# jermp/sshash

Hardware: AMD Instinct MI355X
Metric: k-mer Lookups/sec (batched random queries, bit-exact ids) (higher is better)
Workload: dtype u64

## Files before the change

### sshash_amd/csrc/streaming.hip

```cpp
#include <hip/hip_runtime.h>
#include <sys/stat.h>

#include <algorithm>
#include <atomic>
#include <cstring>
#include <exception>
#include <stdexcept>
#include <thread>

#include "engine.hpp"
#include "hooks.hpp"
#include "reads.hpp"
#include "replica.hpp"
#include "segments.hpp"

namespace sshash_amd {

namespace {

template <int W, bool CANON>
__device__ __forceinline__ hit_t seed_lookup(dict_view const& d, skew_part_dev const* __restrict__ skew,
                                             kmer_w<W> const& x, kmer_w<W> const& x_rc, minimizer_t mf, minimizer_t mr) {
    if constexpr (CANON) {
        if (mf.value < mr.value) return probe_canonical<W, true>(d, skew, x, x_rc, mf);
        if (mr.value < mf.value) return probe_canonical<W, true>(d, skew, x, x_rc, mr);
        hit_t h = probe_canonical<W, true>(d, skew, x, x_rc, mf);
        if (!h.found) h = probe_canonical<W, true>(d, skew, x, x_rc, mr);
        return h;
    } else {
        hit_t h = probe_regular<W, true>(d, skew, x, mf);
        if (!h.found) {
            const bool mf_found = h.minimizer_found;
            h = probe_regular<W, true>(d, skew, x_rc, mr);
            h.orientation = -1;
            h.minimizer_found = h.minimizer_found || mf_found;
        }
        return h;
    }
}

__device__ __forceinline__ uint64_t wave_sum(uint64_t v) {
    for (int o = 32; o > 0; o >>= 1) v += __shfl_down(v, o, 64);
    return v;
}

__device__ __forceinline__ bool continues_run(uint64_t id_before, uint64_t sid_before, int ori_before, uint64_t id, uint64_t sid) {
    return id_before != INVALID_U64 && sid_before == sid && id == id_before + uint64_t(int64_t(ori_before));
}

__device__ __forceinline__ void block_report(uint64_t c_kmers, uint64_t c_invalid, uint64_t c_negative, uint64_t c_searches,
                                             uint64_t c_extensions, uint64_t* __restrict__ report) {
    __shared__ uint64_t partial[4][5];
    c_kmers = wave_sum(c_kmers);
    c_invalid = wave_sum(c_invalid);
    c_negative = wave_sum(c_negative);
    c_searches = wave_sum(c_searches);
    c_extensions = wave_sum(c_extensions);
    if ((threadIdx.x & 63) == 0) {
        uint64_t* mine = partial[threadIdx.x >> 6];
        mine[0] = c_kmers;
        mine[1] = c_invalid;
        mine[2] = c_negative;
        mine[3] = c_searches;
        mine[4] = c_extensions;
    }
    __syncthreads();
    if (threadIdx.x != 0) return;
    uint64_t t[5];
    for (int j = 0; j < 5; ++j) t[j] = partial[0][j] + partial[1][j] + partial[2][j] + partial[3][j];
    if (t[0] == 0) return;
    atomicAdd(reinterpret_cast<unsigned long long*>(report + 0), (unsigned long long)t[0]);
    atomicAdd(reinterpret_cast<unsigned long long*>(report + 1), (unsigned long long)(t[3] + t[4]));
    atomicAdd(reinterpret_cast<unsigned long long*>(report + 2), (unsigned long long)t[2]);
    atomicAdd(reinterpret_cast<unsigned long long*>(report + 3), (unsigned long long)t[1]);
    atomicAdd(reinterpret_cast<unsigned long long*>(report + 4), (unsigned long long)t[3]);
    atomicAdd(reinterpret_cast<unsigned long long*>(report + 5), (unsigned long long)t[4]);
}


__global__ void __launch_bounds__(256)
stream_pack_kernel(const char* __restrict__ bases, const uint64_t total_bases, uint16_t* __restrict__ packed, uint8_t* __restrict__ okay) {
    const uint64_t t = uint64_t(blockIdx.x) * blockDim.x + threadIdx.x;
    const uint64_t at = 8 * t;
    if (at >= total_bases) return;
    uint64_t v = 0;
    if (at + 8 <= total_bases && ((reinterpret_cast<uintptr_t>(bases) + at) & 7) == 0) {
        v = *reinterpret_cast<const uint64_t*>(bases + at);
    } else {
        for (uint32_t b = 0; b < 8 && at + b < total_bases; ++b) v |= uint64_t(uint8_t(bases[at + b])) << (8 * b);
    }
    uint64_t two = (v >> 1) & 0x0303030303030303ULL;
    two = (two | (two >> 6)) & 0x000F000F000F000FULL;
    two = (two | (two >> 12)) & 0x000000FF000000FFULL;
    two = two | (two >> 24);
    const uint64_t u = v & 0xDFDFDFDFDFDFDFDFULL;
    auto nonzero = [](uint64_t z) { return ((z & 0x7F7F7F7F7F7F7F7FULL) + 0x7F7F7F7F7F7F7F7FULL) | z; };
    uint64_t ok = ~(nonzero(u ^ 0x4141414141414141ULL) & nonzero(u ^ 0x4343434343434343ULL) & nonzero(u ^ 0x4747474747474747ULL) &
                    nonzero(u ^ 0x5454545454545454ULL)) & 0x8080808080808080ULL;
    ok >>= 7;
    ok |= ok >> 7;
    ok |= ok >> 14;
    ok |= ok >> 28;
    packed[t] = uint16_t(two);
    okay[t] = uint8_t(ok);
}

__device__ __forceinline__ uint64_t first_invalid_base(const uint64_t* __restrict__ okay, uint64_t from, uint64_t end) {
    uint64_t p = from;
    while (p < end) {
        const uint64_t bad = ~okay[p >> 6] >> (p & 63u);
        if (bad) {
            p += uint64_t(__builtin_ctzll(bad));
            break;
        }
        p = (p | 63u) + 1;
    }
    return p < end ? p : end;
}

__device__ __forceinline__ uint64_t first_valid_base(const uint64_t* __restrict__ okay, uint64_t from, uint64_t end) {
    uint64_t p = from;
    while (p < end) {
        const uint64_t good = okay[p >> 6] >> (p & 63u);
        if (good) {
            p += uint64_t(__builtin_ctzll(good));
            break;
        }
        p = (p | 63u) + 1;
    }
    return p < end ? p : end;
}

__device__ __forceinline__ uint64_t read_bases32(const uint64_t* __restrict__ packed, uint64_t p) {
    const uint64_t i = p >> 5;
    return funnel_shr(packed[i], packed[i + 1], 2 * (uint32_t(p) & 31u));
}

template <int W>
__device__ __forceinline__ void string_bases32(dict_view const& d, uint64_t p, uint64_t& bases, uint64_t& marks) {
    const uint32_t rel = uint32_t(p) & 31u;
    if constexpr (W == 1) {
        const uint4* A = reinterpret_cast<const uint4*>(d.granules) + 2 * (p >> 5);
        const uint4 q0 = A[0], q1 = A[1];
        bases = funnel_shr(uint64_t(q0.x) | (uint64_t(q0.y) << 32), uint64_t(q0.z) | (uint64_t(q0.w) << 32), 2 * rel);
        marks = (uint64_t(q1.x) | (uint64_t(q1.y) << 32)) >> rel;
    } else {
        const uint4* G = reinterpret_cast<const uint4*>(d.granules) + (p >> 5);
        const uint4 g0 = G[0], g1 = G[1];
        bases = funnel_shr(uint64_t(g0.z) | (uint64_t(g0.w) << 32), uint64_t(g1.z) | (uint64_t(g1.w) << 32), 2 * rel);
        marks = (uint64_t(g0.y) | (uint64_t(g1.y) << 32)) >> rel;
    }
}

struct run_step_t {
    uint64_t s, marks, read;
    uint32_t have;
};

template <int W>
__device__ __forceinline__ run_step_t run_step_load(dict_view const& d, const uint64_t* __restrict__ packed, uint64_t off, bool forward,
                                                    uint64_t b, uint64_t run) {
    run_step_t t;
    const uint64_t top = off - run;
    t.have = forward || top >= 32 ? 32u : uint32_t(top);
    string_bases32<W>(d, forward ? off + d.k + run : top - t.have, t.s, t.marks);
    t.read = read_bases32(packed, b + run);
    return t;
}

__device__ __forceinline__ uint32_t run_step_length(run_step_t const& t, bool forward) {
    const uint64_t along = forward ? t.s : revcomp_word(t.s << ((2 * (32 - t.have)) & 63u));
    const uint64_t diff = along ^ t.read;
    const uint32_t same = diff ? uint32_t(__builtin_ctzll(diff)) >> 1 : 32u;
    const uint32_t gate = forward ? uint32_t(__brev(uint32_t(t.marks))) : uint32_t((t.marks >> 1) << (32 - t.have));
    const uint32_t inside = gate ? uint32_t(__builtin_clz(gate)) : 32u;
    const uint32_t step = same < inside ? same : inside;
    return step < t.have ? step : t.have;
}

template <int W>
__device__ __forceinline__ uint64_t extend_run(dict_view const& d, const uint64_t* __restrict__ packed, uint64_t off, int ori, uint64_t b,
                                               uint64_t room, run_step_t t) {
    const bool forward = ori > 0;
    uint64_t run = 0;
    for (;;) {
        uint64_t step = run_step_length(t, forward);
        if (step > room - run) step = room - run;
        run += step;
        if (step < 32 || run >= room) break;
        t = run_step_load<W>(d, packed, off, forward, b, run);
    }
    return run;
}

__device__ __forceinline__ void row_flush(uint64_t* __restrict__ row, bool partial, uint32_t& c_invalid, uint32_t& c_negative, uint32_t& c_searches,
                                          uint32_t& c_extensions) {
    const uint64_t s = c_searches, e = c_extensions;
    if (partial) {
        row[1] += s + e;
        row[2] += c_negative;
        row[3] += c_invalid;
        row[4] += s;
        row[5] += e;
    } else {
        row[1] = s + e;
        row[2] = c_negative;
        row[3] = c_invalid;
        row[4] = s;
        row[5] = e;
    }
    c_invalid = c_negative = c_searches = c_extensions = 0;
}

#ifndef SSHASH_STREAM_WAVES
#define SSHASH_STREAM_WAVES 5
#endif
enum : int { STREAM_TOTALS = 0, STREAM_ROWS = 1, STREAM_RUN_COUNTS = 2, STREAM_RUN_RECORDS = 3, STREAM_COVER = 4, STREAM_DEPTH = 5 };

__device__ __forceinline__ void run_record_store(dict_view const& d, run_sink const& sink, const uint64_t* __restrict__ begins, uint64_t r,
                                                 uint64_t cursor, uint64_t at, uint64_t off, uint32_t sid, int ori, uint64_t n) {
    if (cursor >= sink.capacity || cursor >= sink.run_offsets[r + 1]) return;
    const uint64_t kmer_id = off - uint64_t(sid) * (d.k - 1), in_string = off - d.endpoints[sid];
    const uint32_t read_pos = uint32_t(at - begins[r]), length = uint32_t(n) | (ori > 0 ? 0u : 0x80000000u);
    uint4* const rec = static_cast<uint4*>(sink.records) + 2 * cursor;
    rec[0] = make_uint4(uint32_t(kmer_id), uint32_t(kmer_id >> 32), sid, 0u);
    rec[1] = make_uint4(uint32_t(in_string), uint32_t(in_string >> 32), read_pos, length);
}

__device__ __forceinline__ void cover_mark(uint64_t* __restrict__ cover, uint64_t lo, uint64_t hi) {
    const uint64_t w0 = lo >> 6, w1 = (hi - 1) >> 6;
    const unsigned long long first = ~0ULL << (lo & 63u), last = ~0ULL >> (63u - (uint32_t(hi - 1) & 63u));
    unsigned long long* const words = reinterpret_cast<unsigned long long*>(cover);
    if (w0 == w1) {
        (void)__hip_atomic_fetch_or(words + w0, first & last, __ATOMIC_RELAXED, __HIP_MEMORY_SCOPE_AGENT);
        return;
    }
    (void)__hip_atomic_fetch_or(words + w0, first, __ATOMIC_RELAXED, __HIP_MEMORY_SCOPE_AGENT);
    for (uint64_t w = w0 + 1; w < w1; ++w) words[w] = ~0ULL;
    (void)__hip_atomic_fetch_or(words + w1, last, __ATOMIC_RELAXED, __HIP_MEMORY_SCOPE_AGENT);
}

__device__ __forceinline__ void cover_mark_run(dict_view const& d, run_sink const& sink, uint64_t off, uint32_t sid, int ori, uint64_t n) {
    const uint64_t kmer_id = off - uint64_t(sid) * (d.k - 1);
    const uint64_t lo = ori > 0 ? kmer_id : kmer_id + 1 - n;
    cover_mark(static_cast<uint64_t*>(sink.records), lo, lo + n);
}

__device__ __forceinline__ void depth_mark_run(dict_view const& d, run_sink const& sink, uint64_t off, uint32_t sid, int ori, uint64_t n) {
    const uint64_t kmer_id = off - uint64_t(sid) * (d.k - 1);
    const uint64_t lo = ori > 0 ? kmer_id : kmer_id + 1 - n, hi = lo + n;
    uint32_t* const deltas = static_cast<uint32_t*>(sink.records);
    (void)__hip_atomic_fetch_add(deltas + lo, 1u, __ATOMIC_RELAXED, __HIP_MEMORY_SCOPE_AGENT);
    if (hi < d.num_kmers) (void)__hip_atomic_fetch_add(deltas + hi, ~0u, __ATOMIC_RELAXED, __HIP_MEMORY_SCOPE_AGENT);
}

template <int W, bool CANON, bool SK, int MODE>
__global__ void __launch_bounds__(256, SSHASH_STREAM_WAVES)
streaming_run_kernel(const dict_view d, const skew_part_dev* __restrict__ skew, const uint64_t* __restrict__ packed,
                     const uint64_t* __restrict__ okay, const uint64_t* __restrict__ begins, const uint64_t* __restrict__ ends, const uint64_t n_reads,
                     const uint64_t reads_per_wave, const uint32_t move_out_every, uint64_t* __restrict__ report, const run_sink sink) {
    constexpr bool PER_READ = MODE == STREAM_ROWS, COUNT_RUNS = MODE == STREAM_RUN_COUNTS, RECORDS = MODE == STREAM_RUN_RECORDS, COVER = MODE == STREAM_COVER,
                   DEPTH = MODE == STREAM_DEPTH;
    __shared__ uint4 stage[SK ? 4 * 256 : 1];
    uint4* const wave_stage = stage + (SK ? (threadIdx.x >> 6) * 256 : 0);
    __shared__ unsigned long long moved_out[4][5];
    uint32_t c_invalid = 0, c_negative = 0, c_searches = 0, c_extensions = 0;
    const uint32_t k = d.k;
    const uint32_t lane = threadIdx.x & 63u;
    unsigned long long* const wave_moved_out = moved_out[threadIdx.x >> 6];
    if constexpr (!PER_READ && !RECORDS) {
        if (lane < 5) wave_moved_out[lane] = 0;
    }
    const uint64_t wave = uint64_t(blockIdx.x) * (blockDim.x >> 6) + (threadIdx.x >> 6);
    uint64_t next = wave * reads_per_wave, last = next + reads_per_wave;
    if (next > n_reads) next = n_reads;
    if (last > n_reads) last = n_reads;
    uint64_t cur = 0, rd_end = 0, inv = 0;
    bool pending = false;
    uint64_t off = 0;
    int ori = 1;
    bool neg_unknown_mini = false;
    uint64_t prev_f = 0, prev_r = 0;
    constexpr uint32_t WALK_CHOICE = 7u, WALK_COMPACT = 8u, WALK_VISITED = 16u, WALK_BACK_SHIFT = 8u, WALK_NO_RETURN = 7u;
    constexpr uint32_t WALK_LASTS_SHIFT = 16u, WALK_LASTS = 63u;
    constexpr uint32_t WALK_INLINE = 32u, WALK_HEAVY_BACK_SHIFT = 11u, WALK_HEAVY_SHIFT = 24u, WALK_HEAVY = 63u, WALK_HEAVY_PENDING = 1u << 30;
    constexpr uint32_t WALK_HEAVY_FIELDS = (7u << WALK_HEAVY_BACK_SHIFT) | (WALK_HEAVY << WALK_HEAVY_SHIFT) | WALK_HEAVY_PENDING;
    bool walking = false;
    kmer_w<W> x = kmer_zero<W>(), x_rc = kmer_zero<W>();
    sk_key_t kk{};
    uint64_t on = 0, on_a = 0;
    uint32_t where = 0;
    uint32_t turns = 0;
    constexpr uint32_t ROW_NONE = ~0u, ROW_PARTIAL = 1u << 31;
    uint32_t my_row = ROW_NONE;
    uint32_t n_runs = 0, hit_sid = 0;
    uint64_t cursor = 0;
    const uint64_t wave_first = wave * reads_per_wave;
    uint64_t* const wave_rows = report + wave * reads_per_wave * 6;
#ifdef SSHASH_STREAM_STATS
    unsigned long long st_turns = 0, st_fresh = 0, st_walk = 0, st_ext = 0, st_slot1 = 0, st_inv = 0, st_idle = 0, st_full = 0, st_short = 0;
    uint64_t st_kept_lane = 0;
#define STAT(var, pred) var += (unsigned long long)__popcll(__ballot(pred))
#else
#define STAT(var, pred) (void)0
#endif
    for (;;) {
#ifdef SSHASH_STREAM_STATS
        ++st_turns;
#endif
        if (++turns >= move_out_every) {
            turns = 0;
            if constexpr (PER_READ) {
                if (my_row != ROW_NONE) {
                    row_flush(wave_rows + uint64_t(my_row & ~ROW_PARTIAL) * 6, (my_row & ROW_PARTIAL) != 0, c_invalid, c_negative, c_searches, c_extensions);
                    my_row |= ROW_PARTIAL;
                }
            } else if constexpr (!RECORDS) {
                const uint64_t i = wave_sum(c_invalid), n = wave_sum(c_negative), f = wave_sum(c_searches), e = wave_sum(c_extensions);
                if (lane == 0) {
                    wave_moved_out[0] += i;
                    wave_moved_out[1] += n;
                    wave_moved_out[2] += f;
                    wave_moved_out[3] += e;
                }
                c_invalid = c_negative = c_searches = c_extensions = 0;
            }
        }
        STAT(st_ext, pending);
        if (pending) {
            const uint64_t b = cur + k - 1, valid_end = inv < rd_end ? inv : rd_end;
            const uint64_t run = extend_run<W>(d, packed, off, ori, b, valid_end - b, run_step_load<W>(d, packed, off, ori > 0, b, 0));
            if constexpr (COVER) cover_mark_run(d, sink, off, hit_sid, ori, run + 1);
            if constexpr (DEPTH) depth_mark_run(d, sink, off, hit_sid, ori, run + 1);
            if constexpr (RECORDS) {
                run_record_store(d, sink, begins, wave_first + my_row, cursor, cur - 1, off, hit_sid, ori, run + 1);
                ++cursor;
            } else if (run >> 15) {
                if constexpr (PER_READ) {
                    uint64_t* const row = wave_rows + uint64_t(my_row & ~ROW_PARTIAL) * 6;
                    row_flush(row, (my_row & ROW_PARTIAL) != 0, c_invalid, c_negative, c_searches, c_extensions);
                    my_row |= ROW_PARTIAL;
                    row[1] += run;
                    row[5] += run;
                } else {
                    atomicAdd(wave_moved_out + 3, (unsigned long long)run);
                }
            } else {
                c_extensions += uint32_t(run);
            }
            cur += run;
            if (run) where &= ~WALK_HEAVY_FIELDS;
        }
        pending = false;
        const bool want = !walking && cur + k > rd_end;
        const uint64_t wants = __ballot(want);
        if constexpr (PER_READ) {
            if (want && my_row != ROW_NONE) {
                row_flush(wave_rows + uint64_t(my_row & ~ROW_PARTIAL) * 6, (my_row & ROW_PARTIAL) != 0, c_invalid, c_negative, c_searches, c_extensions);
                my_row = ROW_NONE;
            }
        }
        if constexpr (COUNT_RUNS) {
            if (want && my_row != ROW_NONE) {
                sink.run_offsets[wave_first + my_row] = n_runs;
                n_runs = 0;
                my_row = ROW_NONE;
            }
        }
        if (wants != 0 && next < last) {
            const uint64_t rank = uint64_t(__popcll(wants & ((uint64_t(1) << lane) - 1)));
            if (want && rank < last - next) {
                const uint64_t r = next + rank;
                cur = begins[r];
                rd_end = ends[r];
                if constexpr (PER_READ) {
                    uint64_t* const row = report + r * 6;
                    const uint64_t kmers = rd_end - cur >= k ? rd_end - cur - k + 1 : 0;
                    row[0] = kmers;
                    if (kmers) {
                        my_row = uint32_t(r - wave * reads_per_wave);
                    } else {
                        row[1] = row[2] = row[3] = row[4] = row[5] = 0;
                    }
                } else if constexpr (COUNT_RUNS) {
                    if (rd_end - cur >= k) {
                        atomicAdd(wave_moved_out + 4, (unsigned long long)(rd_end - cur - k + 1));
                        my_row = uint32_t(r - wave_first);
                    } else {
                        sink.run_offsets[r] = 0;
                    }
                } else if constexpr (RECORDS) {
                    my_row = uint32_t(r - wave_first);
                    cursor = sink.run_offsets[r];
                } else {
                    if (rd_end - cur >= k) atomicAdd(wave_moved_out + 4, (unsigned long long)(rd_end - cur - k + 1));
                }
                inv = first_invalid_base(okay, cur, rd_end);
                neg_unknown_mini = false;
                where = 0;
            }
            const uint64_t taken = uint64_t(__popcll(wants));
            next = taken < last - next ? next + taken : last;
        }
        bool live = cur + k <= rd_end;
        if (next >= last && __ballot(live) == 0) break;
        uint32_t c_invalid_turn = 0;
        STAT(st_inv, live && cur + k > inv);
        while (live && cur + k > inv) {
            const uint64_t nv = first_valid_base(okay, inv + 1, rd_end);
            const uint64_t last_over_it = nv - 1 < rd_end - k ? nv - 1 : rd_end - k;
            const uint64_t over = last_over_it - cur + 1;
            if ((over + c_invalid_turn) >> 15) {
                if constexpr (PER_READ) {
                    uint64_t* const row = wave_rows + uint64_t(my_row & ~ROW_PARTIAL) * 6;
                    row_flush(row, (my_row & ROW_PARTIAL) != 0, c_invalid, c_negative, c_searches, c_extensions);
                    my_row |= ROW_PARTIAL;
                    row[3] += over;
                } else if constexpr (!RECORDS) {
                    atomicAdd(wave_moved_out + 0, (unsigned long long)over);
                }
            } else {
                c_invalid_turn += uint32_t(over);
            }
            cur = nv;
            inv = first_invalid_base(okay, nv, rd_end);
            neg_unknown_mini = false;
            where = 0;
            live = cur + k <= rd_end;
        }
        c_invalid += c_invalid_turn;
        const uint64_t valid_end = inv < rd_end ? inv : rd_end;
        uint64_t ahead_f = 0, ahead_r = 0;
        bool table = false;
        STAT(st_fresh, live && !walking);
        STAT(st_walk, live && walking);
        STAT(st_idle, !live);
        if (live && !walking) {
            const uint64_t i = cur >> 5;
            const uint32_t sh = 2 * (uint32_t(cur) & 31u);
            const uint64_t w0 = packed[i], w1 = packed[i + 1];
            x.w[0] = funnel_shr(w0, w1, sh);
            if constexpr (W == 2) x.w[1] = funnel_shr(w1, packed[i + 2], sh);
            x = kmer_take_chars<W>(x, k);
            x_rc = kmer_revcomp<W>(x, k);
            if constexpr (SK) {
                const uint32_t sm = d.sk.m, hashed = sm < 12 ? sm : 12;
                ahead_f = read_bases32(packed, cur + k - sm + 1);
                ahead_r = read_bases32(packed, cur + k + 1 - hashed);
                const uint32_t heavy_left = (where >> WALK_HEAVY_SHIFT) & WALK_HEAVY;
                STAT(st_short, heavy_left != 0);
                if (heavy_left) {
                    kk.pos = kk.rc ? kk.pos + 1 : kk.pos - 1;
                    table = true;
                    on = sk_kmer_key<W>(x, x_rc);
                    const uint32_t back = (where >> WALK_HEAVY_BACK_SHIFT) & 7u;
                    where = WALK_VISITED | WALK_COMPACT | (back << WALK_BACK_SHIFT) | (back << WALK_HEAVY_BACK_SHIFT) | ((heavy_left - 1) << WALK_HEAVY_SHIFT);
                } else {
                    kk = sk_key<W>(x, x_rc, k, sm);
                    table = sk_usable(d, kk);
                    on = kk.key;
                    where = (WALK_NO_RETURN << WALK_BACK_SHIFT) | (WALK_LASTS << WALK_LASTS_SHIFT);
                }
                on_a = sk_hash_a(on);
            }
        }
        if constexpr (SK) {
            if (live && walking && (!(where & WALK_VISITED) || (where & WALK_HEAVY_PENDING))) {
                const uint32_t sm = d.sk.m, hashed = sm < 12 ? sm : 12;
                ahead_f = read_bases32(packed, cur + k - sm + 1);
                ahead_r = read_bases32(packed, cur + k + 1 - hashed);
            }
        }
        bool settled = false, found = false;
        if constexpr (SK) {
            const bool need = table || walking;
            const uint32_t c = where & WALK_CHOICE;
            const bool compact = (where & WALK_COMPACT) != 0;
            uint32_t bucket = 0;
            if (need) bucket = compact ? d.sk.num_buckets + sk_choice_of(on, on_a, c, d.sk.kmer_buckets) : sk_choice_of(on, on_a, c, d.sk.num_buckets);
            sk_stage_lines<W, true>(d, bucket, 0u, need, wave_stage, compact);
            if (need) {
                const uint4* mine = wave_stage + (lane & 3u) * 64 + (lane >> 2) * 4;
                sk_query_t<W> Q = sk_make_query<W>(x, x_rc, kk, uint32_t(on_a) & 0xFFFFFFu);
                fast_t r = fast_unsettled(false);
                sk_bucket_flags flags;
                flags.go_on = 0;
                flags.second_used = false;
                bool marker = false, seen = false, inline_seen = false;
                uint32_t lasts = 0xFFFFu;
                if (!compact) {
                    sk_examine_slot_tracking<W, true, true>(d, Q, c, [mine](uint32_t i) { return mine[i]; }, r, seen, marker, flags, lasts, inline_seen);
                    STAT(st_slot1, r.outcome == FAST_MISS && flags.second_used);
                    if (r.outcome == FAST_MISS && flags.second_used) {
                        if constexpr (W == 1) {
                            sk_examine_slot_tracking<W, false, true>(d, Q, c, [mine](uint32_t i) { return mine[2 + i]; }, r, seen, marker, flags, lasts, inline_seen);
                        } else {
                            const uint4* B1 = reinterpret_cast<const uint4*>(d.sk.slots) + (SK_BUCKET_SLOTS * 2 * W) * uint64_t(bucket) + 2 * W;
                            sk_examine_slot_tracking<W, false, true>(d, Q, c, [B1](uint32_t i) { return B1[i]; }, r, seen, marker, flags, lasts, inline_seen);
                        }
                    }
                } else if constexpr (W == 1) {
                    const uint32_t* words = reinterpret_cast<const uint32_t*>(mine);
                    sk_examine_kmer_line(Q, c, [words](uint32_t i) { return words[i]; }, r, flags);
                } else {
                    sk_examine_kmer_entry<true>(Q, c, [mine](uint32_t i) { return mine[i]; }, r, flags);
                    sk_examine_kmer_entry<false>(Q, c, [mine](uint32_t i) { return mine[2 + i]; }, r, flags);
                }
                {
                    const uint32_t before = (where >> WALK_LASTS_SHIFT) & WALK_LASTS;
                    lasts = lasts < before ? lasts : before;
                    where = (where & ~(WALK_LASTS << WALK_LASTS_SHIFT)) | (lasts << WALK_LASTS_SHIFT) | (inline_seen ? WALK_INLINE : 0u);
                }
                const bool go_on = flags.go_on != 0;
                bool more = false, defer = false;
                if (r.outcome == FAST_MISS) {
                    if (marker && !(where & WALK_VISITED)) {
                        const uint32_t back = go_on ? c + 1 : WALK_NO_RETURN;
                        where = WALK_VISITED | WALK_COMPACT | (back << WALK_BACK_SHIFT) |
                                ((where & WALK_INLINE) ? 0u : (WALK_HEAVY_PENDING | (back << WALK_HEAVY_BACK_SHIFT)));
                        on = sk_kmer_key<W>(x, x_rc);
                        on_a = sk_hash_a(on);
                        more = true;
                    } else if (go_on) {
                        defer = c + 1 >= SK_CHOICES;
                        where = (where & ~WALK_CHOICE) | (c + 1);
                        more = !defer;
                    } else if (compact && ((where >> WALK_BACK_SHIFT) & WALK_CHOICE) != WALK_NO_RETURN) {
                        const uint32_t back = (where >> WALK_BACK_SHIFT) & WALK_CHOICE;
                        defer = back >= SK_CHOICES;
                        where = WALK_VISITED | back | (WALK_NO_RETURN << WALK_BACK_SHIFT) | (where & WALK_HEAVY_FIELDS);
                        on = kk.key;
                        on_a = sk_hash_a(on);
                        more = !defer;
                    }
                }
                walking = more;
                if (!more && !defer) {
                    settled = true;
                    found = r.outcome == FAST_HIT;
                    off = r.kmer_offset;
                    ori = r.orientation;
                    if constexpr (RECORDS || COVER || DEPTH) hit_sid = r.string_id;
                    const bool stands = !found && !(where & WALK_VISITED);
                    if (stands || (where & WALK_HEAVY_PENDING)) {
                        uint64_t keep = sk_key_persists<W>(kk, k, d.sk.m, ahead_f, ahead_r);
                        keep = keep < valid_end - (cur + k) ? keep : valid_end - (cur + k);
                        if (stands) {
                            keep = keep < lasts ? keep : lasts;
                            c_negative += keep;
                            cur += keep;
#ifdef SSHASH_STREAM_STATS
                            st_kept_lane += keep;
#endif
                        } else {
                            where = (where & ~(WALK_HEAVY_PENDING | (WALK_HEAVY << WALK_HEAVY_SHIFT))) | (uint32_t(keep) << WALK_HEAVY_SHIFT);
                        }
                    }
                }
            }
        }
        const bool finishing = live && !walking;
        STAT(st_full, finishing && !settled);
        if (finishing && !settled) {
            const minimizer_t mf = compute_minimizer<W>(x, k, d.m, d.hash_magic);
            const minimizer_t mr = compute_minimizer<W>(x_rc, k, d.m, d.hash_magic);
            if (!SK && neg_unknown_mini && mf.value == prev_f && mr.value == prev_r) {
                found = false;
            } else {
                prev_f = mf.value;
                prev_r = mr.value;
                const hit_t h = seed_lookup<W, CANON>(d, skew, x, x_rc, mf, mr);
                found = h.found;
                off = h.kmer_offset;
                ori = h.orientation;
                if constexpr (RECORDS || COVER || DEPTH) hit_sid = h.string_id;
                neg_unknown_mini = !SK && !h.found && !h.minimizer_found;
            }
        }
        if (finishing) {
            if (found) {
                ++c_searches;
                neg_unknown_mini = false;
                pending = cur + 1 + k <= valid_end;
                if constexpr (COUNT_RUNS) ++n_runs;
                if constexpr (RECORDS) {
                    if (!pending) {
                        run_record_store(d, sink, begins, wave_first + my_row, cursor, cur, off, hit_sid, ori, 1);
                        ++cursor;
                    }
                }
                if constexpr (COVER) {
                    if (!pending) cover_mark_run(d, sink, off, hit_sid, ori, 1);
                }
                if constexpr (DEPTH) {
                    if (!pending) depth_mark_run(d, sink, off, hit_sid, ori, 1);
                }
            } else {
                ++c_negative;
            }
            ++cur;
        }
    }
#ifdef SSHASH_STREAM_STATS
    const unsigned long long st_neg_kept = wave_sum(st_kept_lane);
    if (lane == 0 && MODE == STREAM_TOTALS) {
        unsigned long long* st = reinterpret_cast<unsigned long long*>(report) + 6;
        atomicAdd(st + 0, st_turns); atomicAdd(st + 1, st_fresh); atomicAdd(st + 2, st_walk); atomicAdd(st + 3, st_ext); atomicAdd(st + 4, st_slot1);
        atomicAdd(st + 5, st_inv); atomicAdd(st + 6, st_idle); atomicAdd(st + 7, st_full); atomicAdd(st + 8, st_neg_kept); atomicAdd(st + 9, st_short);
    }
#endif
    if constexpr (PER_READ) {
        if (my_row != ROW_NONE) row_flush(wave_rows + uint64_t(my_row & ~ROW_PARTIAL) * 6, (my_row & ROW_PARTIAL) != 0, c_invalid, c_negative, c_searches, c_extensions);
    } else if constexpr (!RECORDS) {
        if constexpr (COUNT_RUNS) {
            if (my_row != ROW_NONE) sink.run_offsets[wave_first + my_row] = n_runs;
        }
        const bool first = lane == 0;
        block_report(first ? wave_moved_out[4] : 0, uint64_t(c_invalid) + (first ? wave_moved_out[0] : 0), uint64_t(c_negative) + (first ? wave_moved_out[1] : 0),
                     uint64_t(c_searches) + (first ? wave_moved_out[2] : 0), uint64_t(c_extensions) + (first ? wave_moved_out[3] : 0), report);
    }
}

__global__ void __launch_bounds__(256)
stream_rows_sum_kernel(const uint64_t* __restrict__ rows, const uint64_t n_reads, uint64_t* __restrict__ report) {
    uint64_t c_kmers = 0, c_invalid = 0, c_negative = 0, c_searches = 0, c_extensions = 0;
    const uint64_t stride = uint64_t(gridDim.x) * blockDim.x;
    for (uint64_t r = uint64_t(blockIdx.x) * blockDim.x + threadIdx.x; r < n_reads; r += stride) {
        const uint64_t* row = rows + 6 * r;
        c_kmers += row[0];
        c_negative += row[2];
        c_invalid += row[3];
        c_searches += row[4];
        c_extensions += row[5];
    }
    block_report(c_kmers, c_invalid, c_negative, c_searches, c_extensions, report);
}

constexpr uint32_t SCAN_PER_LANE = 16, SCAN_TILE = 256 * SCAN_PER_LANE;
inline uint64_t scan_tiles(uint64_t n) { return (n + SCAN_TILE - 1) / SCAN_TILE; }

template <class T>
__device__ __forceinline__ T block_exclusive_scan(T v, T& total) {
    __shared__ T wave_total[4];
    const uint32_t lane = threadIdx.x & 63u, w = threadIdx.x >> 6;
    T inc = v;
    for (uint32_t o = 1; o < 64; o <<= 1) {
        const T t = __shfl_up(inc, o, 64);
        if (lane >= o) inc += t;
    }
    __syncthreads();
    if (lane == 63) wave_total[w] = inc;
    __syncthreads();
    T before = 0;
    total = 0;
    for (uint32_t j = 0; j < 4; ++j) {
        if (j < w) before += wave_total[j];
        total += wave_total[j];
    }
    return before + inc - v;
}

__global__ void __launch_bounds__(256)
scan_tile_sums_kernel(const uint64_t* __restrict__ data, const uint64_t n, uint64_t* __restrict__ sums) {
    const uint64_t base = uint64_t(blockIdx.x) * SCAN_TILE + threadIdx.x * SCAN_PER_LANE;
    uint64_t v = 0;
    for (uint32_t j = 0; j < SCAN_PER_LANE; ++j)
        if (base + j < n) v += data[base + j];
    uint64_t total;
    block_exclusive_scan(v, total);
    if (threadIdx.x == 0) sums[blockIdx.x] = total;
}

__global__ void __launch_bounds__(256)
scan_sums_kernel(uint64_t* __restrict__ sums, const uint64_t tiles) {
    uint64_t carry = 0;
    for (uint64_t at = 0; at < tiles; at += 256) {
        const uint64_t i = at + threadIdx.x;
        const uint64_t v = i < tiles ? sums[i] : 0;
        uint64_t total;
        const uint64_t before = block_exclusive_scan(v, total);
        if (i < tiles) sums[i] = carry + before;
        carry += total;
    }
}

__global__ void __launch_bounds__(256)
scan_apply_kernel(uint64_t* __restrict__ data, const uint64_t n, const uint64_t* __restrict__ sums) {
    const uint64_t base = uint64_t(blockIdx.x) * SCAN_TILE + threadIdx.x * SCAN_PER_LANE;
    uint64_t e[SCAN_PER_LANE], v = 0;
#pragma unroll
    for (uint32_t j = 0; j < SCAN_PER_LANE; ++j) {
        e[j] = base + j < n ? data[base + j] : 0;
        v += e[j];
    }
    uint64_t total;
    uint64_t at = sums[blockIdx.x] + block_exclusive_scan(v, total);
#pragma unroll
    for (uint32_t j = 0; j < SCAN_PER_LANE; ++j) {
        if (base + j < n) data[base + j] = at;
        at += e[j];
    }
}

void exclusive_scan_u64(uint64_t* data, uint64_t n, uint64_t* sums, hipStream_t s) {
    if (n == 0) return;
    const uint64_t tiles = scan_tiles(n);
    hipLaunchKernelGGL(scan_tile_sums_kernel, dim3(uint32_t(tiles)), dim3(256), 0, s, data, n, sums);
    hipLaunchKernelGGL(scan_sums_kernel, dim3(1), dim3(256), 0, s, sums, tiles);
    hipLaunchKernelGGL(scan_apply_kernel, dim3(uint32_t(tiles)), dim3(256), 0, s, data, n, sums);
    HIP_CHECK(hipGetLastError());
}

__device__ __forceinline__ uint32_t scan_load16_u32(const uint32_t* __restrict__ in, uint64_t base, uint64_t n, bool aligned, uint32_t (&e)[SCAN_PER_LANE]) {
    static_assert(SCAN_PER_LANE == 16, "four 16-byte pieces a lane");
    uint32_t v = 0;
    if (aligned && base + SCAN_PER_LANE <= n) {
        const uint4* const q = reinterpret_cast<const uint4*>(in + base);
#pragma unroll
// ... 128 lines not shown
    if (!report) return;
    const uint64_t in_wave = wave_sum(join ? 1 : 0);
    if ((threadIdx.x & 63u) == 0) wave_joined[threadIdx.x >> 6] = in_wave;
    __syncthreads();
    if (threadIdx.x != 0) return;
    const unsigned long long J = wave_joined[0] + wave_joined[1] + wave_joined[2] + wave_joined[3];
    if (J == 0) return;
    atomicAdd(reinterpret_cast<unsigned long long*>(report + 4), 0ULL - J);
    atomicAdd(reinterpret_cast<unsigned long long*>(report + 5), J);
}

__global__ void __launch_bounds__(256)
stream_segment_rows_kernel(const uint64_t* __restrict__ seg_rows, const uint64_t* __restrict__ seg_read, const uint8_t* __restrict__ joined,
                           const uint64_t* __restrict__ n_segments, const uint64_t bound, uint64_t* __restrict__ rows) {
    const uint64_t g = uint64_t(blockIdx.x) * blockDim.x + threadIdx.x;
    const uint32_t lane = threadIdx.x & 63u;
    const bool has = g < bound && g < *n_segments;
    const uint64_t read = has ? seg_read[g] : SEG_NO_READ;
    uint64_t v[6] = {0, 0, 0, 0, 0, 0};
    if (has) {
#pragma unroll
        for (uint32_t c = 0; c < 6; ++c) v[c] = seg_rows[6 * g + c];
        const uint64_t j = joined[g];
        v[4] -= j;
        v[5] += j;
    }
    if (__ballot(has) == 0) return;
    const uint64_t read_before = __shfl_up(read, 1, 64);
    for (uint32_t o = 1; o < 64; o <<= 1) {
        const bool same = __shfl_down(read, o, 64) == read && lane + o < 64;
#pragma unroll
        for (uint32_t c = 0; c < 6; ++c) {
            const uint64_t further = __shfl_down(v[c], o, 64);
            if (same) v[c] += further;
        }
    }
    if (!has || (lane > 0 && read_before == read)) return;
    unsigned long long* const row = reinterpret_cast<unsigned long long*>(rows + 6 * read);
#pragma unroll
    for (uint32_t c = 0; c < 6; ++c)
        if (v[c]) atomicAdd(row + c, (unsigned long long)v[c]);
}

template <int W, bool CANON>
void launch_seams(device_replica const* rep, dict_view const& d, hipStream_t s, uint64_t const* packed, uint64_t const* okay, uint64_t const* seg_begin,
                  uint64_t const* seg_read, uint64_t const* n_segments, uint64_t bound, uint8_t* joined, uint64_t* report) {
    hipLaunchKernelGGL((stream_seams_kernel<W, CANON>), dim3(uint32_t((bound + 255) / 256)), dim3(256), 0, s, d, rep->d_skew, packed, okay, seg_begin, seg_read,
                       n_segments, bound, joined, report);
    HIP_CHECK(hipGetLastError());
}

template <int MODE>
void launch_run_kernel(device_replica const* rep, dict_view const& d, dim3 grid, dim3 block, hipStream_t s, uint64_t const* packed, uint64_t const* okay,
                       uint64_t const* begins, uint64_t const* ends, uint64_t n_reads, uint64_t reads_per_wave, uint32_t move_out_every, uint64_t* report,
                       run_sink const& sink) {
    auto launch = [&](auto kernel) {
        hipLaunchKernelGGL(kernel, grid, block, 0, s, d, rep->d_skew, packed, okay, begins, ends, n_reads, reads_per_wave, move_out_every, report, sink);
        HIP_CHECK(hipGetLastError());
    };
    const bool wide = d.k > 31, canon = d.canonical, sk = d.sk.enabled;
    if (!wide && !canon && !sk) launch(streaming_run_kernel<1, false, false, MODE>);
    else if (!wide && !canon) launch(streaming_run_kernel<1, false, true, MODE>);
    else if (!wide && !sk) launch(streaming_run_kernel<1, true, false, MODE>);
    else if (!wide) launch(streaming_run_kernel<1, true, true, MODE>);
    else if (!canon && !sk) launch(streaming_run_kernel<2, false, false, MODE>);
    else if (!canon) launch(streaming_run_kernel<2, false, true, MODE>);
    else if (!sk) launch(streaming_run_kernel<2, true, false, MODE>);
    else launch(streaming_run_kernel<2, true, true, MODE>);
}

enum : int { RUNS_COUNT = 1, RUNS_WRITE = 2, RUNS_COVER = 4, RUNS_DEPTH = 8 };
void launch_streaming_runs(device_replica const* rep, char const* bases, uint64_t const* offsets, uint64_t n_reads, uint64_t total_bases, uint64_t* report,
                           hipStream_t s, uint64_t* rows = nullptr ,
                           run_sink sink = run_sink{nullptr, nullptr, 0}, int run_phases = 0,
                           uint64_t S = 0 ) {
    dict_view const& d = rep->view;
    const bool segmented = S != 0;
    if (segmented && (run_phases & (RUNS_COUNT | RUNS_WRITE))) throw error(error_kind::internal, "run records are not segmented");
    segment_layout L{};
    if (segmented) {
        L = segment_scratch(n_reads, total_bases, S, SCAN_TILE, rows != nullptr);
        if (L.words == 0 || (L.bound + 255) / 256 >> 31) throw error(error_kind::argument, "too many segments for one call");
    }
    const uint64_t packed_bytes = ((total_bases + 31) / 32 + 3) * 8, okay_bytes = ((total_bases + 63) / 64 + 2) * 8;
    const uint64_t runs_bytes = run_phases ? (scan_tiles(n_reads + 1) + 6) * 8 : 0;
    uint64_t* const caller_report = report;
    std::lock_guard<std::mutex> sequence(rep->launch_mutex);
    uint64_t* packed = static_cast<uint64_t*>(rep->read_scratch_for(s, packed_bytes + okay_bytes + runs_bytes + L.words * 8));
    uint64_t* okay = packed + packed_bytes / 8;
    uint64_t* scan_sums = okay + okay_bytes / 8;
    uint64_t* const seg = scan_sums + runs_bytes / 8;
    if (total_bases) {
        const uint64_t lanes = (total_bases + 7) / 8;
        hipLaunchKernelGGL(stream_pack_kernel, dim3(uint32_t((lanes + 255) / 256)), dim3(256), 0, s, bases, total_bases,
                           reinterpret_cast<uint16_t*>(packed), reinterpret_cast<uint8_t*>(okay));
    }
    uint64_t const *begins = offsets, *ends = offsets + 1;
    const uint64_t n_whole_reads = n_reads;
    if (segmented) {
        hipLaunchKernelGGL(stream_segment_counts_kernel, dim3(uint32_t((n_reads + 256) / 256)), dim3(256), 0, s, offsets, n_reads, d.k, S, seg + L.first);
        exclusive_scan_u64(seg + L.first, n_reads + 1, seg + L.sums, s);
        hipLaunchKernelGGL(stream_segment_fill_kernel, dim3(uint32_t((L.bound + 255) / 256)), dim3(256), 0, s, offsets, n_reads, seg + L.first, d.k, S, L.bound,
                           seg + L.begin, seg + L.end, seg + L.read);
        HIP_CHECK(hipGetLastError());
        begins = seg + L.begin;
        ends = seg + L.end;
        n_reads = L.bound;
    }
    auto seams = [&](uint8_t* joined, uint64_t* into) {
        uint64_t const* n_segments = seg + L.first + n_whole_reads;
        if (d.k <= 31 && !d.canonical) launch_seams<1, false>(rep, d, s, packed, okay, begins, seg + L.read, n_segments, L.bound, joined, into);
        else if (d.k <= 31) launch_seams<1, true>(rep, d, s, packed, okay, begins, seg + L.read, n_segments, L.bound, joined, into);
        else if (!d.canonical) launch_seams<2, false>(rep, d, s, packed, okay, begins, seg + L.read, n_segments, L.bound, joined, into);
        else launch_seams<2, true>(rep, d, s, packed, okay, begins, seg + L.read, n_segments, L.bound, joined, into);
    };
    const uint64_t max_waves = uint64_t(256) * 4 * SSHASH_STREAM_WAVES;
    uint64_t waves = std::min<uint64_t>(max_waves, std::max<uint64_t>(1, n_reads / (64 * 2)));
    waves = (waves + 3) / 4 * 4;
    const uint64_t reads_per_wave = (n_reads + waves - 1) / waves;
    const dim3 grid(uint32_t(waves / 4)), block(256);
    const uint32_t move_out_every = uint32_t(test_hook_u64("stream_move_out_every", uint64_t(1) << 16, 1, uint64_t(1) << 16));
    auto totals = [&]() {
        if (report) return report;
        uint64_t* spare = scan_sums + scan_tiles(n_whole_reads + 1);
        HIP_CHECK(hipMemsetAsync(spare, 0, 6 * sizeof(uint64_t), s));
        return spare;
    };
    if ((rows || (run_phases & (RUNS_COUNT | RUNS_WRITE))) && reads_per_wave >> 31) throw error(error_kind::argument, "too many reads for one call");
    if (run_phases & RUNS_COVER) {
        launch_run_kernel<STREAM_COVER>(rep, d, grid, block, s, packed, okay, begins, ends, n_reads, reads_per_wave, move_out_every, totals(), sink);
        if (segmented && caller_report) seams(nullptr, caller_report);
    } else if (run_phases & RUNS_DEPTH) {
        launch_run_kernel<STREAM_DEPTH>(rep, d, grid, block, s, packed, okay, begins, ends, n_reads, reads_per_wave, move_out_every, totals(), sink);
        if (segmented && caller_report) seams(nullptr, caller_report);
    } else if (run_phases) {
        if (run_phases & RUNS_COUNT) {
            launch_run_kernel<STREAM_RUN_COUNTS>(rep, d, grid, block, s, packed, okay, begins, ends, n_reads, reads_per_wave, move_out_every, totals(), sink);
            HIP_CHECK(hipMemsetAsync(sink.run_offsets + n_reads, 0, sizeof(uint64_t), s));
            exclusive_scan_u64(sink.run_offsets, n_reads + 1, scan_sums, s);
        }
        if (run_phases & RUNS_WRITE)
            launch_run_kernel<STREAM_RUN_RECORDS>(rep, d, grid, block, s, packed, okay, begins, ends, n_reads, reads_per_wave, move_out_every, nullptr, sink);
    } else if (rows) {
        if (segmented) {
            uint8_t* const joined = reinterpret_cast<uint8_t*>(seg + L.joined);
            launch_run_kernel<STREAM_ROWS>(rep, d, grid, block, s, packed, okay, begins, ends, n_reads, reads_per_wave, move_out_every, seg + L.rows, sink);
            seams(joined, nullptr);
            HIP_CHECK(hipMemsetAsync(rows, 0, n_whole_reads * 6 * sizeof(uint64_t), s));
            hipLaunchKernelGGL(stream_segment_rows_kernel, dim3(uint32_t((L.bound + 255) / 256)), dim3(256), 0, s, seg + L.rows, seg + L.read, joined,
                               seg + L.first + n_whole_reads, L.bound, rows);
            HIP_CHECK(hipGetLastError());
        } else {
            launch_run_kernel<STREAM_ROWS>(rep, d, grid, block, s, packed, okay, begins, ends, n_reads, reads_per_wave, move_out_every, rows, sink);
        }
        if (report) {
            const uint32_t blocks = uint32_t(std::min<uint64_t>((n_whole_reads + 255) / 256, 1024));
            hipLaunchKernelGGL(stream_rows_sum_kernel, dim3(blocks), dim3(256), 0, s, rows, n_whole_reads, report);
            HIP_CHECK(hipGetLastError());
        }
    } else {
        launch_run_kernel<STREAM_TOTALS>(rep, d, grid, block, s, packed, okay, begins, ends, n_reads, reads_per_wave, move_out_every, report, sink);
        if (segmented && report) seams(nullptr, report);
    }
}

uint64_t resolve_total_bases(uint64_t const* d_read_offsets, uint64_t n_reads, uint64_t total_bases, hipStream_t s) {
    if (n_reads && total_bases == 0) {
// ... 186 lines not shown
        end = ends[lo];
        begin = lo ? ends[lo - 1] : offsets[r0];
    } else {
        uint64_t a = r0, b = n_reads - 1;
        while (a < b) {
            const uint64_t mid = a + (b - a + 1) / 2;
            if (offsets[mid] <= p) a = mid;
            else b = mid - 1;
        }
        begin = offsets[a];
        end = offsets[a + 1];
    }
    uint8_t f = 0;
    kmer_w<W> x = kmer_zero<W>();
    if (end != ~uint64_t(0) && p + k <= end) {
        const uint32_t cw = tid >> 4, cs = 2 * (tid & 15u);
        uint32_t word[2 * W];
        for (int j = 0; j < 2 * W; ++j) word[j] = __builtin_amdgcn_alignbit(codes[cw + j + 1], codes[cw + j], cs);
        for (int j = 0; j < W; ++j) x.w[j] = uint64_t(word[2 * j]) | (uint64_t(word[2 * j + 1]) << 32);
        x = kmer_take_chars<W>(x, k);
        const uint32_t vw = tid >> 5, vs = tid & 31u;
        const uint64_t ok = uint64_t(__builtin_amdgcn_alignbit(okay[vw + 1], okay[vw], vs)) |
                            (uint64_t(__builtin_amdgcn_alignbit(okay[vw + 2], okay[vw + 1], vs)) << 32);
        const bool valid = (~ok & low_mask(k)) == 0;
        f = (valid ? SQ_VALID : SQ_INVALID) | (p == begin ? SQ_FIRST : 0);
    }
    flags[p] = f;
    for (int j = 0; j < W; ++j) kmers[(p - first) * W + j] = x.w[j];
}

__global__ void __launch_bounds__(256)
stream_classify_kernel(const uint8_t* __restrict__ flags, const uint64_t total_bases, const result_view out,
                       const uint64_t* string_id, const int8_t* orientation , uint64_t* __restrict__ report,
                       const bool has_predecessor ) {
    uint64_t c_kmer = 0, c_invalid = 0, c_negative = 0, c_search = 0, c_extension = 0;
    constexpr uint32_t PLACES = 4;
    const uint64_t stride = uint64_t(gridDim.x) * blockDim.x * PLACES;
    for (uint64_t p0 = (uint64_t(blockIdx.x) * blockDim.x + threadIdx.x) * PLACES; p0 < total_bases; p0 += stride) {
        const int64_t q = (p0 || has_predecessor) ? int64_t(p0) - 1 : 0;
        uint8_t f[PLACES + 1];
        uint64_t id[PLACES + 1], sid[PLACES + 1];
        int8_t ori[PLACES + 1];
        f[0] = flags[q];
        id[0] = out.kmer_id[q];
        sid[0] = string_id[q];
        ori[0] = orientation[q];
        const bool whole = p0 + PLACES <= total_bases && ((reinterpret_cast<uintptr_t>(flags) + p0) & 3) == 0;
        const uint32_t four = whole ? *reinterpret_cast<const uint32_t*>(flags + p0) : 0u;
#pragma unroll
        for (uint32_t j = 0; j < PLACES; ++j) {
            const uint64_t p = p0 + j < total_bases ? p0 + j : total_bases - 1;
            f[j + 1] = whole ? uint8_t(four >> (8 * j)) : flags[p];
            id[j + 1] = out.kmer_id[p];
            sid[j + 1] = string_id[p];
            ori[j + 1] = orientation[p];
        }
#pragma unroll
        for (uint32_t j = 0; j < PLACES; ++j) {
            const uint64_t p = p0 + j;
            if (p >= total_bases) break;
            if (f[j + 1] & SQ_INVALID) {
                ++c_kmer;
                ++c_invalid;
                out.kmer_id[p] = INVALID_U64;
                if (out.kmer_id_in_string) out.kmer_id_in_string[p] = INVALID_U64;
                if (out.kmer_offset) out.kmer_offset[p] = INVALID_U64;
                if (out.string_id) out.string_id[p] = INVALID_U64;
                if (out.string_begin) out.string_begin[p] = INVALID_U64;
                if (out.string_end) out.string_end[p] = INVALID_U64;
                if (out.kmer_orientation) out.kmer_orientation[p] = 1;
            } else if (f[j + 1] & SQ_VALID) {
                ++c_kmer;
                if (id[j + 1] == INVALID_U64) {
                    ++c_negative;
                } else {
                    const bool extension = !(f[j + 1] & SQ_FIRST) && (f[j] & SQ_VALID) && continues_run(id[j], sid[j], ori[j], id[j + 1], sid[j + 1]);
                    c_extension += extension;
                    c_search += !extension;
                }
            }
        }
    }
    if (!report) return;
    block_report(c_kmer, c_invalid, c_negative, c_search, c_extension, report);
}

__global__ void __launch_bounds__(256)
stream_classify_rows_kernel(const uint8_t* __restrict__ flags, const uint64_t total_bases, const uint64_t* __restrict__ kmer_id,
                            const uint64_t* __restrict__ string_id, const int8_t* __restrict__ orientation,
                            const uint64_t* __restrict__ offsets, const uint64_t n_reads, uint64_t* __restrict__ rows) {
    const uint64_t p = uint64_t(blockIdx.x) * blockDim.x + threadIdx.x;
    const uint32_t lane = threadIdx.x & 63u;
    const uint8_t f = p < total_bases ? flags[p] : uint8_t(0);
    const bool has = (f & (SQ_VALID | SQ_INVALID)) != 0, invalid = (f & SQ_INVALID) != 0;
    bool negative = false, search = false, extension = false;
    if (!invalid && (f & SQ_VALID)) {
        const uint64_t id = kmer_id[p];
        if (id == INVALID_U64) {
            negative = true;
        } else {
            if (!(f & SQ_FIRST) && p > 0 && (flags[p - 1] & SQ_VALID)) {
                extension = continues_run(kmer_id[p - 1], string_id[p - 1], orientation[p - 1], id, string_id[p]);
            }
            search = !extension;
        }
    }
    const uint64_t have = __ballot(has);
    if (have == 0) return;
    const uint64_t below = (uint64_t(1) << lane) - 1;
    const bool head = has && ((f & SQ_FIRST) || (have & below) == 0);
    const uint64_t heads = __ballot(head);
    const uint64_t m_invalid = __ballot(invalid), m_negative = __ballot(negative), m_search = __ballot(search), m_extension = __ballot(extension);
    if (!head) return;
    const uint64_t above = (heads >> lane) >> 1;
    const uint32_t end = above ? lane + 1 + uint32_t(__builtin_ctzll(above)) : 64u;
    const uint64_t mine = (end == 64 ? ~uint64_t(0) : (uint64_t(1) << end) - 1) & ~below;
    uint64_t lo = 0, hi = n_reads - 1;
    while (lo < hi) {
        const uint64_t mid = lo + (hi - lo + 1) / 2;
        if (offsets[mid] <= p) lo = mid;
        else hi = mid - 1;
    }
    unsigned long long* const row = reinterpret_cast<unsigned long long*>(rows + 6 * lo);
    const unsigned long long n_kmers = __popcll(have & mine), n_invalid = __popcll(m_invalid & mine), n_negative = __popcll(m_negative & mine),
                             n_search = __popcll(m_search & mine), n_extension = __popcll(m_extension & mine);
    atomicAdd(row + 0, n_kmers);
    if (n_search + n_extension) atomicAdd(row + 1, n_search + n_extension);
    if (n_negative) atomicAdd(row + 2, n_negative);
    if (n_invalid) atomicAdd(row + 3, n_invalid);
    if (n_search) atomicAdd(row + 4, n_search);
    if (n_extension) atomicAdd(row + 5, n_extension);
}

constexpr uint8_t RUN_HEAD = 1, RUN_CONTINUES = 2;

__global__ void __launch_bounds__(256)
stream_run_marks_kernel(const uint8_t* __restrict__ flags, const uint64_t total_bases, const uint64_t* __restrict__ kmer_id,
                        const uint64_t* __restrict__ string_id, const int8_t* __restrict__ orientation, uint8_t* __restrict__ marks ,
                        uint64_t* __restrict__ rank ) {
    const uint64_t p = uint64_t(blockIdx.x) * blockDim.x + threadIdx.x;
    if (p > total_bases) return;
    uint8_t mark = 0;
    if (p < total_bases) {
        const uint8_t f = flags[p];
        if (!(f & SQ_INVALID) && (f & SQ_VALID)) {
            const uint64_t id = kmer_id[p];
            if (id != INVALID_U64) {
                bool extension = false;
                if (!(f & SQ_FIRST) && p > 0 && (flags[p - 1] & SQ_VALID)) {
                    extension = continues_run(kmer_id[p - 1], string_id[p - 1], orientation[p - 1], id, string_id[p]);
                }
                mark = extension ? RUN_CONTINUES : RUN_HEAD;
            }
        }
    }
    marks[p] = mark;
    rank[p] = mark == RUN_HEAD ? 1 : 0;
}

__global__ void __launch_bounds__(256)
stream_run_offsets_kernel(const uint64_t* __restrict__ rank, const uint64_t total_bases, const uint64_t* __restrict__ offsets, const uint64_t n_reads,
                          uint64_t* __restrict__ run_offsets) {
    const uint64_t r = uint64_t(blockIdx.x) * blockDim.x + threadIdx.x;
    if (r > n_reads) return;
    const uint64_t at = offsets[r];
    run_offsets[r] = rank[at < total_bases ? at : total_bases];
}
// ... 710 lines not shown
```

Baseline: 41.01 billion.

## Cache a per-lane window of packed read words in LDS for streaming lookups

Each lane keeps a seven-word window of packed read bases in shared memory, loaded when a read opens or the cursor jumps, and serves k-mer, lookahead and run-extension reads from it instead of global memory. The window open also scans the validity bitmap from registers before falling back to the global search. Scratch buffers are padded so the window loads stay in bounds, and block_report now takes a caller-provided shared array so the streaming kernel can reuse its moved_out buffer. The trade is more LDS per block, which the static_assert limits to keep the configured waves per SIMD, plus extra bookkeeping on every step.

New measurement: 41.02 billion, median of 2. Within noise of the previous version (+0.0%).

```diff
diff --git a/sshash_amd/csrc/streaming.hip b/sshash_amd/csrc/streaming.hip
--- a/sshash_amd/csrc/streaming.hip
+++ b/sshash_amd/csrc/streaming.hip
@@ -49,15 +49,14 @@
 }
 
 __device__ __forceinline__ void block_report(uint64_t c_kmers, uint64_t c_invalid, uint64_t c_negative, uint64_t c_searches,
-                                             uint64_t c_extensions, uint64_t* __restrict__ report) {
-    __shared__ uint64_t partial[4][5];
+                                             uint64_t c_extensions, uint64_t* __restrict__ report, unsigned long long (*partial)[5]) {
     c_kmers = wave_sum(c_kmers);
     c_invalid = wave_sum(c_invalid);
     c_negative = wave_sum(c_negative);
     c_searches = wave_sum(c_searches);
     c_extensions = wave_sum(c_extensions);
     if ((threadIdx.x & 63) == 0) {
-        uint64_t* mine = partial[threadIdx.x >> 6];
+        unsigned long long* mine = partial[threadIdx.x >> 6];
         mine[0] = c_kmers;
         mine[1] = c_invalid;
         mine[2] = c_negative;
@@ -131,9 +130,75 @@
     return p < end ? p : end;
 }
 
-__device__ __forceinline__ uint64_t read_bases32(const uint64_t* __restrict__ packed, uint64_t p) {
-    const uint64_t i = p >> 5;
-    return funnel_shr(packed[i], packed[i + 1], 2 * (uint32_t(p) & 31u));
+constexpr uint32_t READ_WINDOW = 7;
+template <int W>
+constexpr uint32_t READ_SPAN = W + 2;
+constexpr uint32_t WINDOW_OKAY = (READ_WINDOW * 32 + 32 + 63) / 64;
+struct read_window_t {
+    uint64_t words[READ_WINDOW][256];
+    uint32_t from[256];
+};
+
+__device__ __forceinline__ void window_store(read_window_t& window, uint32_t col, const uint64_t (&w)[READ_WINDOW], uint64_t word) {
+#pragma unroll
+    for (uint32_t j = 0; j < READ_WINDOW; ++j) window.words[j][col] = w[j];
+    window.from[col] = uint32_t(word);
+}
+
+template <int W>
+__device__ __forceinline__ uint32_t window_seek(read_window_t& window, uint32_t col, const uint64_t* __restrict__ packed, uint64_t word) {
+    static_assert(READ_SPAN<W> <= READ_WINDOW, "a seed's words fit the window");
+    const uint32_t from = window.from[col];
+    if (uint32_t(word) - from <= READ_WINDOW - READ_SPAN<W>) return from;
+    uint64_t w[READ_WINDOW];
+#pragma unroll
+    for (uint32_t j = 0; j < READ_WINDOW; ++j) w[j] = packed[word + j];
+    window_store(window, col, w, word);
+    return uint32_t(word);
+}
+
+__device__ __forceinline__ void window_far(read_window_t& window, uint32_t col, uint64_t moved, uint64_t p) {
+    if (moved >> 31) window.from[col] = uint32_t(p >> 5) + 0x80000000u;
+}
+
+__device__ __forceinline__ uint64_t window_open(read_window_t& window, uint32_t col, const uint64_t* __restrict__ packed, const uint64_t* __restrict__ okay,
+                                                uint64_t cur, uint64_t rd_end) {
+    const uint64_t* const words = packed + (cur >> 5);
+    const uint64_t* const valid = okay + (cur >> 6);
+    uint64_t w[READ_WINDOW], ok[WINDOW_OKAY];
+#pragma unroll
+    for (uint32_t j = 0; j < READ_WINDOW; ++j) w[j] = words[j];
+#pragma unroll
+    for (uint32_t j = 0; j < WINDOW_OKAY; ++j) ok[j] = valid[j];
+    window_store(window, col, w, cur >> 5);
+    uint64_t p = cur;
+    bool met = false;
+#pragma unroll
+    for (uint32_t j = 0; j < WINDOW_OKAY; ++j) {
+        if (!met && p < rd_end) {
+            const uint64_t bad = ~ok[j] >> (p & 63u);
+            met = bad != 0;
+            p = met ? p + uint64_t(__builtin_ctzll(bad)) : (p | 63u) + 1;
+        }
+    }
+    if (!met && p < rd_end) return first_invalid_base(okay, p, rd_end);
+    return p < rd_end ? p : rd_end;
+}
+
+__device__ __forceinline__ uint64_t window_bases32(const read_window_t& window, uint32_t col, uint32_t from, uint64_t p) {
+    const uint32_t j = uint32_t(p >> 5) - from;
+    return funnel_shr(window.words[j][col], window.words[j + 1][col], 2 * (uint32_t(p) & 31u));
+}
+
+template <int W>
+__device__ __forceinline__ kmer_w<W> window_kmer_words(const read_window_t& window, uint32_t col, uint32_t from, uint64_t p) {
+    const uint32_t j = uint32_t(p >> 5) - from;
+    const uint32_t sh = 2 * (uint32_t(p) & 31u);
+    const uint64_t w0 = window.words[j][col], w1 = window.words[j + 1][col];
+    kmer_w<W> x = kmer_zero<W>();
+    x.w[0] = funnel_shr(w0, w1, sh);
+    if constexpr (W == 2) x.w[1] = funnel_shr(w1, window.words[j + 2][col], sh);
+    return x;
 }
 
 template <int W>
@@ -158,13 +223,14 @@
 };
 
 template <int W>
-__device__ __forceinline__ run_step_t run_step_load(dict_view const& d, const uint64_t* __restrict__ packed, uint64_t off, bool forward,
+__device__ __forceinline__ run_step_t run_step_load(dict_view const& d, const uint64_t* __restrict__ packed, read_window_t& window, uint32_t col, uint64_t off, bool forward,
                                                     uint64_t b, uint64_t run) {
     run_step_t t;
     const uint64_t top = off - run;
     t.have = forward || top >= 32 ? 32u : uint32_t(top);
+    const uint32_t from = window_seek<W>(window, col, packed, (b + run - (d.k - 1)) >> 5);
     string_bases32<W>(d, forward ? off + d.k + run : top - t.have, t.s, t.marks);
-    t.read = read_bases32(packed, b + run);
+    t.read = window_bases32(window, col, from, b + run);
     return t;
 }
 
@@ -179,16 +245,16 @@
 }
 
 template <int W>
-__device__ __forceinline__ uint64_t extend_run(dict_view const& d, const uint64_t* __restrict__ packed, uint64_t off, int ori, uint64_t b,
-                                               uint64_t room, run_step_t t) {
+__device__ __forceinline__ uint64_t extend_run(dict_view const& d, const uint64_t* __restrict__ packed, read_window_t& window, uint32_t col, uint64_t off, int ori,
+                                               uint64_t b, uint64_t room) {
     const bool forward = ori > 0;
     uint64_t run = 0;
     for (;;) {
+        const run_step_t t = run_step_load<W>(d, packed, window, col, off, forward, b, run);
         uint64_t step = run_step_length(t, forward);
         if (step > room - run) step = room - run;
         run += step;
         if (step < 32 || run >= room) break;
-        t = run_step_load<W>(d, packed, off, forward, b, run);
     }
     return run;
 }
@@ -262,16 +328,22 @@
     constexpr bool PER_READ = MODE == STREAM_ROWS, COUNT_RUNS = MODE == STREAM_RUN_COUNTS, RECORDS = MODE == STREAM_RUN_RECORDS, COVER = MODE == STREAM_COVER,
                    DEPTH = MODE == STREAM_DEPTH;
     __shared__ uint4 stage[SK ? 4 * 256 : 1];
-    uint4* const wave_stage = stage + (SK ? (threadIdx.x >> 6) * 256 : 0);
+    const uint32_t wave_in_group = __builtin_amdgcn_readfirstlane(threadIdx.x >> 6);
+    uint4* const wave_stage = stage + (SK ? wave_in_group * 256 : 0);
     __shared__ unsigned long long moved_out[4][5];
+    __shared__ read_window_t window;
+    constexpr size_t LDS_PIECE = 1280, LDS_PIECES = 160 * 1024 / LDS_PIECE;
+    static_assert((4 * 256 * sizeof(uint4) + sizeof(moved_out) + sizeof(read_window_t) + LDS_PIECE - 1) / LDS_PIECE <= LDS_PIECES / SSHASH_STREAM_WAVES,
+                  "the read window costs the kernel a wave a SIMD");
     uint32_t c_invalid = 0, c_negative = 0, c_searches = 0, c_extensions = 0;
     const uint32_t k = d.k;
     const uint32_t lane = threadIdx.x & 63u;
-    unsigned long long* const wave_moved_out = moved_out[threadIdx.x >> 6];
+    unsigned long long* const wave_moved_out = moved_out[wave_in_group];
+    const uint32_t col = wave_in_group * 64 + lane;
     if constexpr (!PER_READ && !RECORDS) {
         if (lane < 5) wave_moved_out[lane] = 0;
     }
-    const uint64_t wave = uint64_t(blockIdx.x) * (blockDim.x >> 6) + (threadIdx.x >> 6);
+    const uint64_t wave = uint64_t(blockIdx.x) * (blockDim.x >> 6) + wave_in_group;
     uint64_t next = wave * reads_per_wave, last = next + reads_per_wave;
     if (next > n_reads) next = n_reads;
     if (last > n_reads) last = n_reads;
@@ -285,6 +357,7 @@
     constexpr uint32_t WALK_LASTS_SHIFT = 16u, WALK_LASTS = 63u;
     constexpr uint32_t WALK_INLINE = 32u, WALK_HEAVY_BACK_SHIFT = 11u, WALK_HEAVY_SHIFT = 24u, WALK_HEAVY = 63u, WALK_HEAVY_PENDING = 1u << 30;
     constexpr uint32_t WALK_HEAVY_FIELDS = (7u << WALK_HEAVY_BACK_SHIFT) | (WALK_HEAVY << WALK_HEAVY_SHIFT) | WALK_HEAVY_PENDING;
+    static_assert(SK_PERSIST_MAX <= WALK_HEAVY, "how long a heavy key lasts (sk_key_persists) fits its field of `where`");
     bool walking = false;
     kmer_w<W> x = kmer_zero<W>(), x_rc = kmer_zero<W>();
     sk_key_t kk{};
@@ -329,7 +402,7 @@
         STAT(st_ext, pending);
         if (pending) {
             const uint64_t b = cur + k - 1, valid_end = inv < rd_end ? inv : rd_end;
-            const uint64_t run = extend_run<W>(d, packed, off, ori, b, valid_end - b, run_step_load<W>(d, packed, off, ori > 0, b, 0));
+            const uint64_t run = extend_run<W>(d, packed, window, col, off, ori, b, valid_end - b);
             if constexpr (COVER) cover_mark_run(d, sink, off, hit_sid, ori, run + 1);
             if constexpr (DEPTH) depth_mark_run(d, sink, off, hit_sid, ori, run + 1);
             if constexpr (RECORDS) {
@@ -395,7 +468,7 @@
                 } else {
                     if (rd_end - cur >= k) atomicAdd(wave_moved_out + 4, (unsigned long long)(rd_end - cur - k + 1));
                 }
-                inv = first_invalid_base(okay, cur, rd_end);
+                inv = window_open(window, col, packed, okay, cur, rd_end);
                 neg_unknown_mini = false;
                 where = 0;
             }
@@ -422,6 +495,7 @@
             } else {
                 c_invalid_turn += uint32_t(over);
             }
+            window_far(window, col, nv - cur, nv);
             cur = nv;
             inv = first_invalid_base(okay, nv, rd_end);
             neg_unknown_mini = false;
@@ -435,18 +509,15 @@
         STAT(st_fresh, live && !walking);
         STAT(st_walk, live && walking);
         STAT(st_idle, !live);
+        uint32_t win_from = 0;
+        if (live) win_from = window_seek<W>(window, col, packed, cur >> 5);
         if (live && !walking) {
-            const uint64_t i = cur >> 5;
-            const uint32_t sh = 2 * (uint32_t(cur) & 31u);
-            const uint64_t w0 = packed[i], w1 = packed[i + 1];
-            x.w[0] = funnel_shr(w0, w1, sh);
-            if constexpr (W == 2) x.w[1] = funnel_shr(w1, packed[i + 2], sh);
-            x = kmer_take_chars<W>(x, k);
+            x = kmer_take_chars<W>(window_kmer_words<W>(window, col, win_from, cur), k);
             x_rc = kmer_revcomp<W>(x, k);
             if constexpr (SK) {
                 const uint32_t sm = d.sk.m, hashed = sm < 12 ? sm : 12;
-                ahead_f = read_bases32(packed, cur + k - sm + 1);
-                ahead_r = read_bases32(packed, cur + k + 1 - hashed);
+                ahead_f = window_bases32(window, col, win_from, cur + k - sm + 1);
+                ahead_r = window_bases32(window, col, win_from, cur + k + 1 - hashed);
                 const uint32_t heavy_left = (where >> WALK_HEAVY_SHIFT) & WALK_HEAVY;
                 STAT(st_short, heavy_left != 0);
                 if (heavy_left) {
@@ -467,8 +538,8 @@
         if constexpr (SK) {
             if (live && walking && (!(where & WALK_VISITED) || (where & WALK_HEAVY_PENDING))) {
                 const uint32_t sm = d.sk.m, hashed = sm < 12 ? sm : 12;
-                ahead_f = read_bases32(packed, cur + k - sm + 1);
-                ahead_r = read_bases32(packed, cur + k + 1 - hashed);
+                ahead_f = window_bases32(window, col, win_from, cur + k - sm + 1);
+                ahead_r = window_bases32(window, col, win_from, cur + k + 1 - hashed);
             }
         }
         bool settled = false, found = false;
@@ -617,7 +688,7 @@
         }
         const bool first = lane == 0;
         block_report(first ? wave_moved_out[4] : 0, uint64_t(c_invalid) + (first ? wave_moved_out[0] : 0), uint64_t(c_negative) + (first ? wave_moved_out[1] : 0),
-                     uint64_t(c_searches) + (first ? wave_moved_out[2] : 0), uint64_t(c_extensions) + (first ? wave_moved_out[3] : 0), report);
+                     uint64_t(c_searches) + (first ? wave_moved_out[2] : 0), uint64_t(c_extensions) + (first ? wave_moved_out[3] : 0), report, moved_out);
     }
 }
 
@@ -633,7 +704,8 @@
         c_searches += row[4];
         c_extensions += row[5];
     }
-    block_report(c_kmers, c_invalid, c_negative, c_searches, c_extensions, report);
+    __shared__ unsigned long long partial[4][5];
+    block_report(c_kmers, c_invalid, c_negative, c_searches, c_extensions, report, partial);
 }
 
 constexpr uint32_t SCAN_PER_LANE = 16, SCAN_TILE = 256 * SCAN_PER_LANE;
@@ -928,7 +1000,8 @@
         L = segment_scratch(n_reads, total_bases, S, SCAN_TILE, rows != nullptr);
         if (L.words == 0 || (L.bound + 255) / 256 >> 31) throw error(error_kind::argument, "too many segments for one call");
     }
-    const uint64_t packed_bytes = ((total_bases + 31) / 32 + 3) * 8, okay_bytes = ((total_bases + 63) / 64 + 2) * 8;
+    static_assert(READ_WINDOW >= 3, "the seam kernel reads up to two words past a k-mer's first");
+    const uint64_t packed_bytes = (total_bases / 32 + READ_WINDOW) * 8, okay_bytes = (total_bases / 64 + WINDOW_OKAY) * 8;
     const uint64_t runs_bytes = run_phases ? (scan_tiles(n_reads + 1) + 6) * 8 : 0;
     uint64_t* const caller_report = report;
     std::lock_guard<std::mutex> sequence(rep->launch_mutex);
@@ -1281,7 +1354,8 @@
         }
     }
     if (!report) return;
-    block_report(c_kmer, c_invalid, c_negative, c_search, c_extension, report);
+    __shared__ unsigned long long partial[4][5];
+    block_report(c_kmer, c_invalid, c_negative, c_search, c_extension, report, partial);
 }
 
 __global__ void __launch_bounds__(256)
```
